# ztaylor797/APMBackend

Measured on AMD Instinct MI355X. Metric: log-lines/sec z-scored (whole node), higher is better.
Workload: dtype fp64

## Files before the change

### apmbackend_amd/csrc/bindings.cpp

```cpp
#include <pybind11/pybind11.h>
#include <pybind11/stl.h>

#include <cstring>
#include <memory>

#include "kernels/kernel_api.h"
#include "runtime/engine.h"
#include "runtime/format.h"
#include "runtime/jsutil.h"
#include "runtime/merge.h"

namespace apm {
namespace copyenc {
void encode_blob(std::string_view blob, std::string* out, int64_t* counts);
}
int apm_txcopy_lines(const char* d_text, const uint64_t* h_line_off, int64_t n, std::string& out_rows);
std::vector<double> apm_release_bench(int64_t n, int iters, uint64_t seed);
}

namespace py = pybind11;
using namespace apm;

void register_tailer(py::module_& m);
void register_synth(py::module_& m);
// ... 759 lines not shown
  m.def("js_parse_int", [](const std::string& s) { return js::parse_int(s); });
  m.def("js_convert_date", [](const std::string& s, const py::dict& tz) {
    double v;
    TzTable t = tz_from(tz);
    if (!js::convert_date(s, t, v)) return py::object(py::none());
    return py::object(py::float_(v));
  });
  m.def("js_round_fixed", [](double x, int f) { return js_round_fixed(x, f); });
  m.def("hist_bin", [](int32_t v) { return hist_bin(v); });
  m.def("hist_lower", [](int b) { return hist_lower(b); });
  m.def("hist_group_max", []() { return apm_hist_group_max(); });
  m.def("winpct_group_max", []() { return apm_winpct_group_max(); });
  m.def("winpct_group_win", []() { return apm_winpct_group_win(); });
  m.def("slo_group_max", []() { return apm_slo_group_max(); });
  m.def("slo_stage_bytes", []() { return apm_slo_stage_bytes(); });

  register_tailer(m);
  register_synth(m);
  register_procstat(m);
  register_dbsink(m);
}
```

### apmbackend_amd/csrc/kernels/devjoin.hip

```cpp
#include "kernel_api.h"

#include <rocprim/rocprim.hpp>

#include <chrono>
#include <climits>
#include <cstdlib>
#include <cstddef>
#include <cstring>
#include <vector>

#include "devjoin_api.h"
#include "devjoin_dev.h"
#include "devscan.h"
#include "prim.h"
#include "textout.h"

namespace apm {
using namespace dj;

namespace {

constexpr int TB = 256;

__device__ __forceinline__ uint32_t grid_n(uint32_t n) { return (n + TB - 1) / TB; }
// ... 2271 lines not shown
}
static int dj_scan_bucket_max(PrimScratch& sc, const int64_t* bucket, int64_t* bmax, size_t n, hipStream_t s) {
  return prim_inclusive_scan(sc, bucket, bmax, n, rocprim::maximum<int64_t>(), s);
}

size_t apm_dj_tmp_bytes(uint32_t max_ev, uint32_t max_out) {
  PrimScratch q;
  const size_t n = std::max<size_t>(max_ev, 1) + 1;
  dj_sort_keys(q, nullptr, nullptr, nullptr, nullptr, n, 0);
  dj_scan_counts(q, nullptr, nullptr, n, 0);
  dj_scan_lens(q, nullptr, nullptr, (size_t)max_out + 1, 0);
  dj_scan_bucket_max(q, nullptr, nullptr, (size_t)max_out + 1, 0);
  return q.need + 4096;
}

int apm_dj_select_host(DJArgs* a, const uint32_t* d_n_ev, uint32_t max_ev, hipStream_t s) {
  HIP_OK(hipMemsetAsync(a->n_host, 0, sizeof(SelCount), s));
  if (max_ev == 0) return 0;
  uint32_t* list = reinterpret_cast<uint32_t*>(a->sel_pos);
  uint32_t* list_n = list + max_ev;
  HIP_OK(hipMemsetAsync(list_n, 0, 8, s));
  const dim3 grid((max_ev + TB - 1) / TB);
  hipLaunchKernelGGL(k_host_flags, grid, dim3(TB), 0, s, a->ev, d_n_ev, a->bytes, a->host_flag, a->sel_val, a->aud,
                     a->n_host, max_ev, list, list_n);
  dj_check(s, "k_host_flags");
  hipLaunchKernelGGL(k_host_flags_bytes, grid, dim3(TB), 0, s, a->ev, a->bytes, a->chunk_file, a->file_fkey,
                     a->host_flag, a->sel_val, a->aud, max_ev, list, list_n);
  dj_check(s, "k_host_flags_bytes");
  uint64_t* total = a->sel_pos + (max_ev + DS_TILE - 1) / DS_TILE + 1;
  if (ds_scan_apply<uint64_t>(SelValF{a->sel_val},
                              SelScatterG{a->ev, a->host_flag, total, a->host_ev, a->host_ev_idx, a->mh_idx,
                                          a->walk_idx, a->n_host},
                              d_n_ev, max_ev, a->sel_pos, total, s) != 0)
    return -1;
  dj_check(s, "k_ds_scan (host selection)");
  return 0;
// ... 337 lines not shown
```

### apmbackend_amd/csrc/kernels/devjoin_api.h

```cpp
#pragma once
#include <vector>
#include <hip/hip_runtime.h>
#include <stdint.h>

#include "../apm_types.h"
#include "devjoin_types.h"

namespace apm {

constexpr int SOAP_SEGS = 16;
constexpr uint32_t DJ_OVF_CAP = 1u << 16;

enum : uint32_t {
  DJ_WRITE_OK = 0,
  DJ_WRITE_TXT = 1,
  DJ_WRITE_TOO_BIG = 2,
  DJ_WRITE_RING_FULL = 3,
};

__host__ __device__ inline uint64_t ring_place(uint64_t head, uint64_t bytes, uint64_t cap) {
  return ((head & (cap - 1)) + bytes > cap) ? (head + cap - 1) & ~(cap - 1) : head;
}

struct DJOverflow {
// ... 138 lines not shown
  uint32_t* unresolved;
  char* txt_tx;
  char* txt_db;
  int want_tx, want_db;
  JoinCounts* counts;
  void* tmp;
  size_t tmp_bytes;
};

}

extern "C" {
size_t apm_dj_tmp_bytes(uint32_t max_ev, uint32_t max_out);
int apm_dj_take_marks(double* t, const char** names, int cap);
void apm_dj_gather_field(const void* base, size_t stride, uint32_t n, int words, uint32_t* out, hipStream_t s);
int apm_dj_select_host(apm::DJArgs* a, const uint32_t* d_n_ev, uint32_t max_ev, hipStream_t s);
int apm_dj_join(apm::DJArgs* a, hipStream_t s);
int apm_dj_plan(apm::DJFormatArgs* f, hipStream_t s);
int apm_dj_write(apm::DJFormatArgs* f, hipStream_t s);
void apm_dj_rebuild(const apm::KeyState* old, uint32_t old_cap, apm::KeyState* fresh, uint32_t fresh_mask,
                    const apm::NeedEnt* arena, uint32_t arena_cap, double now, apm::JoinCounts* counts,
                    unsigned long long* live, uint8_t* pool, uint32_t* pool_ring, uint32_t pool_mask, hipStream_t s);
size_t apm_dj_rebuild_scratch_bytes(uint32_t cap);
std::vector<double> apm_dj_rebuild_selftest(uint32_t cap, double load, double dead, uint64_t seed, bool copy);
void apm_dj_rebuild_inplace(apm::KeyState* table, uint32_t cap, uint32_t* scratch, const apm::NeedEnt* arena,
                            uint32_t arena_cap, double now, apm::JoinCounts* counts, unsigned long long* live,
                            uint8_t* pool, uint32_t* pool_ring, uint32_t pool_mask, hipStream_t s);
size_t apm_dj_live_tmp_bytes(uint32_t cap);
void apm_dj_live_compact(const apm::KeyState* table, uint32_t cap, apm::KeyState* out, uint32_t* d_n, void* tmp,
                         size_t tmp_bytes, hipStream_t s);
void apm_dj_gather_blocks(const uint8_t* pool, const int32_t* idx, uint32_t n, uint8_t* out, hipStream_t s);
// ... 28 lines not shown
```

### apmbackend_amd/csrc/kernels/kernel_api.h

```cpp
#pragma once
#include <hip/hip_runtime.h>
#include <stdint.h>

#include "../apm_types.h"
#include "common.h"

namespace apm {

struct StatsState {
  int32_t* counts;
  int32_t* cells;
  int32_t* spill_n;
  int32_t* spill_series;
  int32_t* spill_val;
  uint8_t* active;
  int32_t cap;
  int32_t spill_cap;
  int32_t S;
  int32_t nslot = NSLOT_MIN;
  unsigned long long* spill_drop = nullptr;
  int32_t* nan_until = nullptr;
  int32_t* ord_list = nullptr;
  int32_t* ord_n = nullptr;
  uint32_t* ord_done = nullptr;
// ... 62 lines not shown
};

struct CopySeg {
  void* dst;
  const void* src;
  size_t bytes;
};
struct CopySegs {
  CopySeg seg[8];
  int32_t n = 0;
  void add(void* d, const void* s, size_t b) {
    if (b) seg[n++] = CopySeg{d, s, b};
  }
};

struct ExportArgs {
  static constexpr int kMax = 8;
  void* src[kMax];
  void* dst[kMax];
  uint64_t reset_val[kMax];
  uint8_t bytes[kMax];
  uint8_t reset[kMax];
  int32_t n;
  void add(void* s, void* d, int nb, bool rst = false, uint64_t rv = 0) {
    src[n] = s; dst[n] = d; bytes[n] = (uint8_t)nb; reset[n] = rst ? 1 : 0; reset_val[n] = rv; ++n;
  }
};

struct FormatArgs {
  const int32_t* perm;
// ... 124 lines not shown
  int32_t both_only;
  int32_t max_out;
  const double* cool_t;
  double now;
  double cool_s;
};

}

extern "C" {
size_t apm_parse_workspace_bytes(uint64_t max_bytes, uint32_t max_lines, uint32_t max_chunks);
int apm_parse_batch(const uint8_t* d_bytes, uint64_t n_bytes, const uint32_t* d_chunk_begin,
                    const uint8_t* d_chunk_kind, const uint32_t* d_chunk_file, uint32_t n_chunks,
                    void* d_ws, uint32_t max_lines, apm::Event* d_events, uint32_t* d_n_events,
                    uint32_t* d_n_lines, unsigned long long* d_watermark, uint8_t* d_file_open,
                    const apm::TzTable* tz, hipStream_t stream);
size_t apm_ck_pack_tmp_bytes(uint64_t n_entries);
int apm_ck_pack_cells(const int32_t* counts, const int32_t* cells, const int32_t* d_slots, int k, int32_t n, int32_t S,
                      int32_t cap, uint32_t* lens, uint32_t* offs, void* tmp, size_t tmp_bytes, int32_t* packed,
                      hipStream_t s);
void apm_stats_clear_slot(apm::StatsState* st, int slot, hipStream_t stream);
void apm_bucket_append(const apm::TxRec* d_tx, uint32_t lo, uint32_t hi, apm::StatsState* st,
                       int64_t min_live_bucket, hipStream_t stream);
void apm_nan_mark(const apm::TxRec* d_tx, uint32_t n, apm::StatsState* st, hipStream_t stream);
void apm_window_stats(apm::WindowArgs* a, hipStream_t stream);
size_t apm_spill_sort_tmp_bytes(int32_t spill_cap, int32_t S, int32_t nslot);
int apm_spill_sort(const apm::StatsState* st, int32_t* series_out, int32_t* val_out, void* tmp, size_t tmp_bytes,
                   hipStream_t stream);
void apm_pool_append(const apm::TxRec* d_tx, uint32_t lo, uint32_t hi, const int64_t* d_gid, int64_t* tail_end,
                     int64_t* tail_gid, int64_t base, hipStream_t stream);
size_t apm_release_tmp_bytes(int64_t cap);
// ... 56 lines not shown
```

### apmbackend_amd/csrc/kernels/parse.hip

```cpp
#include "kernel_api.h"

#include "prim.h"

#include "devscan.h"

#include <algorithm>
#include <cstdio>
#include <cstdlib>
#include <cstring>

namespace apm {

constexpr int NL_BLOCK = 256;
constexpr int NL_TILE = NL_BLOCK * 16;
constexpr int PARSE_BLOCK = 256;
constexpr int PARSE_LDS = 32 * 1024;

constexpr int NL_PER = 4;

__device__ __forceinline__ uint32_t nl_count16(const uint4 v) {
  const uint32_t w[4] = {v.x, v.y, v.z, v.w};
  uint32_t c = 0;
#pragma unroll
  for (int k = 0; k < 4; ++k) {
    const uint32_t x = w[k] ^ 0x0a0a0a0aU;
    const uint32_t t = ~(((x & 0x7F7F7F7Fu) + 0x7F7F7F7Fu) | x | 0x7F7F7F7Fu);
    c += __popc(t);
  }
  return c;
}

__global__ __launch_bounds__(NL_BLOCK) void k_nl_count(const uint8_t* __restrict__ bytes, uint64_t n,
                                                      uint32_t* __restrict__ tile_counts, uint8_t* __restrict__ pad,
                                                      uint32_t tiles) {
  if (blockIdx.x == 0 && threadIdx.x < 64) pad[threadIdx.x] = 0;
  if (blockIdx.x == 0 && threadIdx.x == 64) tile_counts[tiles] = 0;
  uint4 v[NL_PER];
  uint64_t base[NL_PER];
#pragma unroll
  for (int k = 0; k < NL_PER; ++k) {
    base[k] = ((uint64_t)blockIdx.x * NL_PER + k) * NL_TILE + threadIdx.x * 16;
    if (base[k] + 16 <= n) v[k] = *reinterpret_cast<const uint4*>(bytes + base[k]);
  }
  uint32_t pk[NL_PER / 2] = {0, 0};
#pragma unroll
  for (int k = 0; k < NL_PER; ++k) {
    uint32_t c = 0;
    if (base[k] + 16 <= n) {
      c = nl_count16(v[k]);
    } else {
      for (uint64_t i = base[k]; i < n && i < base[k] + 16; ++i) c += bytes[i] == '\n';
// ... 2 lines not shown
  }
  __shared__ uint32_t red[NL_PER / 2][NL_BLOCK / APM_WAVE];
#pragma unroll
  for (int h = 0; h < NL_PER / 2; ++h) {
    uint32_t c = pk[h];
    for (int o = 32; o > 0; o >>= 1) c += __shfl_down(c, o, APM_WAVE);
    if ((threadIdx.x & 63) == 0) red[h][threadIdx.x >> 6] = c;
  }
  __syncthreads();
  if (threadIdx.x < NL_PER) {
    const int k = threadIdx.x;
    uint32_t sum = 0;
    for (int i = 0; i < NL_BLOCK / APM_WAVE; ++i) sum += red[k >> 1][i];
    const uint32_t tile = blockIdx.x * NL_PER + k;
    if (tile < tiles) tile_counts[tile] = (sum >> (16 * (k & 1))) & 0xFFFFu;
  }
}

__global__ __launch_bounds__(NL_BLOCK) void k_nl_write(const uint8_t* __restrict__ bytes, uint64_t n,
                                                      const uint32_t* __restrict__ tile_off,
                                                      uint32_t* __restrict__ line_end, uint32_t* __restrict__ n_lines,
                                                      uint32_t tiles) {
  if (blockIdx.x == 0 && threadIdx.x == 0) *n_lines = tile_off[tiles];
  uint4 v[NL_PER];
#pragma unroll
  for (int k = 0; k < NL_PER; ++k) {
    const uint64_t base = ((uint64_t)blockIdx.x * NL_PER + k) * NL_TILE + threadIdx.x * 16;
    v[k] = base + 16 <= n ? *reinterpret_cast<const uint4*>(bytes + base) : make_uint4(0, 0, 0, 0);
  }
  typedef rocprim::block_scan<int, NL_BLOCK> Scan;
// ... 941 lines not shown
  __device__ uint32_t operator()(uint32_t i) const { return keep[i]; }
};
struct CompactG {
  const uint8_t* keep;
  const Event* ev_tmp;
  Event* out;
  __device__ void operator()(uint32_t i, uint32_t p) const {
    if (keep[i]) out[p] = ev_tmp[i];
  }
};

}

extern "C" {

constexpr size_t APM_SCAN_TMP = 32u << 20;

size_t apm_parse_workspace_bytes(uint64_t max_bytes, uint32_t max_lines, uint32_t max_chunks) {
  using namespace apm;
  const uint64_t tiles = (max_bytes + NL_TILE - 1) / NL_TILE + 2;
  size_t b = 0;
  b += tiles * 8 + 64;
  b += (size_t)max_lines * (4 + 4 + 4 + 1) + 64;
  b += (size_t)max_lines * sizeof(Event) + 64;
  b += (size_t)(max_chunks + 2) * 4 + 256;
  b += (size_t)(max_chunks + 2) * (SEC_SEGS + 1) + 256;
  b += APM_SCAN_TMP;
  return b;
}

int apm_parse_batch(const uint8_t* d_bytes, uint64_t n_bytes, const uint32_t* d_chunk_begin,
                    const uint8_t* d_chunk_kind, const uint32_t* d_chunk_file, uint32_t n_chunks,
                    void* d_ws, uint32_t max_lines, apm::Event* d_events, uint32_t* d_n_events,
                    uint32_t* d_n_lines, unsigned long long* d_watermark, uint8_t* d_file_open,
                    const apm::TzTable* tz, hipStream_t stream) {
  using namespace apm;
  const uint32_t tiles = (uint32_t)((n_bytes + NL_TILE - 1) / NL_TILE);
  if (tiles == 0 || n_chunks == 0) {
    HIP_OK(hipMemsetAsync(d_n_events, 0, 4, stream));
    HIP_OK(hipMemsetAsync(d_n_lines, 0, 4, stream));
    HIP_OK(hipMemsetAsync(const_cast<uint8_t*>(d_bytes) + n_bytes, 0, 64, stream));
    return 0;
  }
  const uint32_t cap = (uint32_t)std::min<uint64_t>(max_lines, n_bytes);
  uint8_t* w = (uint8_t*)d_ws;
  auto carve = [&](size_t bytes) { uint8_t* r = (uint8_t*)(((uintptr_t)w + 63) & ~(uintptr_t)63); w = r + bytes; return r; };
  uint32_t* tile_counts = (uint32_t*)carve((size_t)(tiles + 1) * 4);
  uint32_t* tile_off = (uint32_t*)carve((size_t)(tiles + 1) * 4);
  uint32_t* line_end = (uint32_t*)carve((size_t)max_lines * 4);
  Event* ev_tmp = (Event*)carve((size_t)max_lines * sizeof(Event));
  uint32_t* line_mask = (uint32_t*)carve((size_t)max_lines * 4);
  uint32_t* pos = (uint32_t*)carve((size_t)max_lines * 4);
  uint8_t* keep = carve((size_t)max_lines);
  uint32_t* chunk_line_lo = (uint32_t*)carve((size_t)(n_chunks + 2) * 4);
  uint8_t* seg_state = carve((size_t)(n_chunks + 2) * SEC_SEGS);
  uint8_t* chunk_init = carve((size_t)(n_chunks + 2));
  void* scan_tmp = carve(APM_SCAN_TMP);

  const uint32_t nl_blocks = (tiles + NL_PER - 1) / NL_PER;
  hipLaunchKernelGGL(k_nl_count, dim3(nl_blocks), dim3(NL_BLOCK), 0, stream, d_bytes, n_bytes, tile_counts,
                     const_cast<uint8_t*>(d_bytes) + n_bytes, tiles);
  PrimScratch sc(scan_tmp, APM_SCAN_TMP);
  if (prim_exclusive_scan(sc, tile_counts, tile_off, 0u, (size_t)tiles + 1, rocprim::plus<uint32_t>(), stream) != 0)
    return -1;
  hipLaunchKernelGGL(k_nl_write, dim3(nl_blocks), dim3(NL_BLOCK), 0, stream, d_bytes, n_bytes, tile_off, line_end,
                     d_n_lines, tiles);

  ParseArgs pa;
  pa.bytes = d_bytes;
  pa.line_end = line_end;
  pa.chunk_begin = d_chunk_begin;
  pa.chunk_kind = d_chunk_kind;
  pa.n_lines_dev = d_n_lines;
  pa.cap_lines = cap;
  pa.n_chunks = n_chunks;
  pa.ev_tmp = ev_tmp;
  pa.line_mask = line_mask;
  pa.keep = keep;
  pa.watermark = d_watermark;
// ... 25 lines not shown
            h[PP_COOP] ? (double)h[PP_HEAD] / h[PP_COOP] : 0.0, h[PP_COOP] ? (double)h[PP_TAIL] / h[PP_COOP] : 0.0);
  }
  hipLaunchKernelGGL(k_chunk_lines, dim3((n_chunks + 1 + 255) / 256), dim3(256), 0, stream, d_chunk_begin,
                     n_chunks, line_end, d_n_lines, chunk_line_lo, tile_off, tiles);
  hipLaunchKernelGGL(k_section_summary, dim3(n_chunks, SEC_SEGS), dim3(APM_WAVE), 0, stream, chunk_line_lo,
                     d_chunk_kind, d_chunk_file, n_chunks, line_mask, d_file_open, seg_state, chunk_init);
  hipLaunchKernelGGL(k_section_apply, dim3(n_chunks, SEC_SEGS), dim3(APM_WAVE), 0, stream, chunk_line_lo,
                     d_chunk_kind, d_chunk_file, n_chunks, line_mask, keep, ev_tmp, d_file_open, seg_state,
                     chunk_init);
  if (ds_scan_apply<uint32_t>(KeepF{keep}, CompactG{keep, ev_tmp, d_events}, d_n_lines, cap, pos, d_n_events,
                              stream) != 0)
    return -1;
  return 0;
}

}
```

### apmbackend_amd/csrc/runtime/devjoin.cpp

```cpp
#include "devjoin.h"

#include <algorithm>
#include <chrono>
#include <climits>
#include <cstddef>
#include <cstdlib>
#include <cstring>
#include <stdexcept>

#include "../kernels/common.h"
#include "binio.h"
#include "d2h.h"
#include "../kernels/devjoin_dev.h"
#include "../kernels/kernel_api.h"
#include "join_util.h"
#include "jsutil.h"

namespace apm {

using namespace jstr;

namespace {
double clock_ms() {
  return std::chrono::duration<double, std::milli>(std::chrono::steady_clock::now().time_since_epoch()).count();
// ... 38 lines not shown
    s.host_flag = (uint8_t*)res_.dmalloc_on(stream_, E + 64);
    s.d_host_ev = (Event*)res_.dmalloc_on(stream_, (size_t)E * sizeof(Event));
    s.d_host_idx = (uint32_t*)res_.dmalloc_on(stream_, (size_t)E * 4);
    s.d_mh_idx = (uint32_t*)res_.dmalloc_on(stream_, (size_t)E * 4);
    s.d_walk_idx = (uint32_t*)res_.dmalloc_on(stream_, (size_t)E * 4);
    s.d_aud = (AudF*)res_.dmalloc_on(stream_, (size_t)E * sizeof(AudF));
    s.d_n_host = (SelCount*)res_.dmalloc_on(stream_, 64);
    res_.pin(s.h_host_ev, (size_t)E * sizeof(Event));
    res_.pin(s.h_host_idx, (size_t)E * 4);
    res_.pin(s.h_n_host, 64);
    std::memset(s.h_n_host, 0, 64);
    s.d_chunk_next = (int32_t*)res_.dmalloc_on(stream_, ((size_t)cfg_.max_chunks + 2) * 4);
    s.d_chunk_first = (uint8_t*)res_.dmalloc_on(stream_, (size_t)cfg_.max_chunks + 2);
    res_.pin(s.h_chunk_next, ((size_t)cfg_.max_chunks + 2) * 4);
    res_.pin(s.h_chunk_first, (size_t)cfg_.max_chunks + 2);
    s.d_tx = (TxRec*)res_.dmalloc_on(stream_, (size_t)out_cap_ * sizeof(TxRec));
    s.d_tx_raw = (int32_t*)res_.dmalloc_on(stream_, (size_t)out_cap_ * 4);
    s.d_tx_gid = (int64_t*)res_.dmalloc_on(stream_, (size_t)out_cap_ * 8);
    s.free_ev = res_.new_event();
  }
  table_cap_ = 1u << cfg_.table_bits;
  init_table_cap_ = table_cap_;
  init_arena_cap_ = cfg_.arena_cap;
  d_table_ = (KeyState*)res_.dmalloc_on(stream_, (size_t)table_cap_ * sizeof(KeyState));
  d_reg_ = (RegSlot*)res_.dmalloc_on(stream_, ((size_t)1 << cfg_.reg_bits) * sizeof(RegSlot));
  miss_cap_ = E;
  d_miss_ = (RegMiss*)res_.dmalloc_on(stream_, (size_t)miss_cap_ * sizeof(RegMiss));
  res_.pin(h_miss_, (size_t)miss_cap_ * sizeof(RegMiss));
  d_arena_ = (NeedEnt*)res_.dmalloc_on(stream_, (size_t)cfg_.arena_cap * sizeof(NeedEnt));
  d_exp_lo_ = (uint64_t*)res_.dmalloc_on(stream_, 8 * 4096);
// ... 97 lines not shown
  const size_t n = files_->size();
  if (n <= h_file_fkey_.size()) return;
  if (n > soap_cap_) throw std::runtime_error("device join: too many files");
  const size_t lo = h_file_fkey_.size();
  if (lo == 0) HIP_OK(hipStreamSynchronize(stream_));
  for (size_t i = lo; i < n; ++i) {
    const FileInfo& f = (*files_)[i];
    const std::string& srv = (*servers_)[f.server];
    h_file_skey_.push_back(dj::server_key_of(srv.data(), srv.size()));
    h_file_fkey_.push_back(dj::file_key_of(f.path.data(), f.path.size()));
  }
  HIP_OK(hipMemcpy(d_file_skey_ + lo, h_file_skey_.data() + lo, (n - lo) * 8, hipMemcpyHostToDevice));
  HIP_OK(hipMemcpy(d_file_fkey_ + lo, h_file_fkey_.data() + lo, (n - lo) * 8, hipMemcpyHostToDevice));
}

void DeviceJoin::select_host(int k, const uint32_t* d_n_ev, uint32_t max_ev, hipStream_t ps) {
  Slot& s = sl_[k];
  sync_file_keys();
  DJArgs a{};
  a.ev = s.d_events;
  a.bytes = s.d_bytes;
  a.host_flag = s.host_flag;
  a.chunk_file = s.d_chunk_file;
  a.file_fkey = d_file_fkey_;
  a.aud = s.d_aud;
  a.sel_val = d_sel_val_;
  a.sel_pos = d_sel_pos_;
  a.host_ev = s.d_host_ev;
  a.host_ev_idx = s.d_host_idx;
  a.mh_idx = s.d_mh_idx;
  a.walk_idx = s.d_walk_idx;
  a.n_host = s.d_n_host;
  a.tmp = d_sel_tmp_;
  a.tmp_bytes = sel_tmp_bytes_;
  if (apm_dj_select_host(&a, d_n_ev, std::min<uint32_t>(max_ev, cfg_.max_events), ps) != 0)
    throw std::runtime_error("device join: scan scratch too small");
  HIP_OK(hipMemcpyAsync(s.h_n_host, s.d_n_host, sizeof(SelCount), hipMemcpyDeviceToHost, ps));
  s.spec = std::min<uint32_t>(cfg_.max_events, last_host_ + last_host_ / 4 + 256);
  HIP_OK(hipMemcpyAsync(s.h_host_ev, s.d_host_ev, (size_t)s.spec * sizeof(Event), hipMemcpyDeviceToHost, ps));
  HIP_OK(hipMemcpyAsync(s.h_host_idx, s.d_host_idx, (size_t)s.spec * 4, hipMemcpyDeviceToHost, ps));
}

void DeviceJoin::set_chunks(int k, const std::vector<int32_t>& chunk_file, const uint32_t* d_chunk_file,
                            const uint8_t* d_chunk_kind, hipStream_t ps) {
  Slot& s = sl_[k];
  const uint32_t n = (uint32_t)chunk_file.size();
  std::unordered_map<int32_t, int32_t> last;
  for (uint32_t c = 0; c < n; ++c) {
    s.h_chunk_next[c] = -1;
    auto it = last.find(chunk_file[c]);
    if (it == last.end()) {
      s.h_chunk_first[c] = 1;
    } else {
      s.h_chunk_first[c] = 0;
      s.h_chunk_next[it->second] = (int32_t)c;
    }
    last[chunk_file[c]] = (int32_t)c;
  }
  if (n) {
    HIP_OK(hipMemcpyAsync(s.d_chunk_next, s.h_chunk_next, (size_t)n * 4, hipMemcpyHostToDevice, ps));
    HIP_OK(hipMemcpyAsync(s.d_chunk_first, s.h_chunk_first, n, hipMemcpyHostToDevice, ps));
  }
  s.d_chunk_file = d_chunk_file;
  s.d_chunk_kind = d_chunk_kind;
  s.n_chunks = n;
  s.chunk_file = chunk_file;
}

void DeviceJoin::finish_select(int k, hipStream_t ps) {
  Slot& s = sl_[k];
  const uint32_t n = s.h_n_host->host;
  if (n > s.spec) {
    HIP_OK(hipMemcpyAsync(s.h_host_ev + s.spec, s.d_host_ev + s.spec, (size_t)(n - s.spec) * sizeof(Event),
                          hipMemcpyDeviceToHost, ps));
    HIP_OK(hipMemcpyAsync(s.h_host_idx + s.spec, s.d_host_idx + s.spec, (size_t)(n - s.spec) * 4,
                          hipMemcpyDeviceToHost, ps));
    HIP_OK(hipStreamSynchronize(ps));
// ... 572 lines not shown
  spans.clear();
  double sp = phase_t[1];
  auto span = [&](const char* name) { const double t = clock_ms(); spans.push_back({name, {sp, t}}); sp = t; };
  res_.reserve(h_hops_, hops_.size(), hops_.size() * 2 + 65536, true);
  res_.reserve(h_hbuf_, hbuf_.size(), hbuf_.size() * 2 + (4 << 20), true);
  span("u.hostgrow");
  if (hops_.size() > d_hops_cap_) {
    d_hops_cap_ = hops_.size() * 2 + 65536;
    d_hops_ = (HostOp*)res_.dmalloc_raw(d_hops_cap_ * sizeof(HostOp));
  }
  if (hbuf_.size() > d_hbuf_cap_) {
    d_hbuf_cap_ = hbuf_.size() * 2 + (4 << 20);
    d_hbuf_ = (uint8_t*)res_.dmalloc_raw(d_hbuf_cap_);
  }
  span("u.devgrow");
  if (!hops_.empty()) {
    std::memcpy(h_hops_, hops_.data(), hops_.size() * sizeof(HostOp));
    span("u.hops.memcpy");
    apm_copy(d_hops_, h_hops_.d, hops_.size() * sizeof(HostOp), st);
    span("u.hops.h2d");
  }
  if (!hbuf_.empty()) {
    std::memcpy(h_hbuf_, hbuf_.data(), hbuf_.size());
    span("u.hbuf.memcpy");
    apm_copy(d_hbuf_, h_hbuf_.d, hbuf_.size(), st);
    span("u.hbuf.h2d");
  }
  sync_file_keys();
  if (files_->size() > files_uploaded_) {
    if (files_->size() > soap_cap_) throw std::runtime_error("device join: too many files");
    std::vector<int32_t> fs(files_->size() - files_uploaded_);
    for (size_t i = files_uploaded_; i < files_->size(); ++i) fs[i - files_uploaded_] = (*files_)[i].server;
    HIP_OK(hipMemcpyAsync(d_file_server_ + files_uploaded_, fs.data(), fs.size() * 4, hipMemcpyHostToDevice, st));
    HIP_OK(hipStreamSynchronize(st));
    files_uploaded_ = files_->size();
  }
  ensure_capacity(n_ev, n_bytes + hbuf_.size(), now);
  span("u.capacity");
  const uint64_t arena_low = regions_.empty() ? arena_head_ : regions_.front().lo;
  const uint32_t arena_limit = (uint32_t)((uint64_t)cfg_.arena_cap - (arena_head_ - arena_low));
  uint32_t n_reg = 0, n_exp = 0;
  while (!regions_.empty() && regions_.front().exp < now && n_reg < 4096) {
    h_exp_[n_reg] = regions_.front().lo;
    h_exp_[4096 + n_reg] = regions_.front().hi;
    n_exp += (uint32_t)(regions_.front().hi - regions_.front().lo);
    regions_.pop_front();
    ++n_reg;
  }
  if (n_reg) {
    apm_copy(d_exp_lo_, h_exp_.d, (size_t)n_reg * 8, st);
    apm_copy(d_exp_hi_, (const uint64_t*)h_exp_.d + 4096, (size_t)n_reg * 8, st);
  }
  span("u.files+exp");
  DJArgs& a = a_;
  a = DJArgs{};
  a.ev = s.d_events; a.n_ev = n_ev; a.bytes = s.d_bytes;
  a.chunk_file = s.d_chunk_file; a.chunk_kind = s.d_chunk_kind; a.n_chunks = s.n_chunks;
  a.chunk_next = s.d_chunk_next; a.chunk_first = s.d_chunk_first; a.file_server = d_file_server_;
  a.file_skey = d_file_skey_; a.file_fkey = d_file_fkey_;
  a.hops = d_hops_; a.n_hops = (uint32_t)hops_.size(); a.hbuf = d_hbuf_;
  a.now = now; a.batch_no = batch_no;
  a.rec_ttl = cfg_.record_ttl_ms; a.acct_ttl = cfg_.acct_ttl_ms; a.need_ttl = cfg_.need_ttl_ms;
  a.host_flag = s.host_flag;
  a.ops = d_ops_; a.soap_code = d_soap_code_; a.soap_num = d_soap_num_; a.soap_hash = d_soap_hash_;
  a.chunk_ev_lo = d_chunk_ev_lo_; a.seg_f = d_seg_f_; a.seg_in = d_seg_in_; a.chain_hash = d_chain_hash_;
  a.soap_state = d_soap_;
  a.op_slot = d_op_slot_; a.op_slot_sorted = d_op_slot_sorted_; a.op_idx = d_op_idx_; a.op_idx_sorted = d_op_idx_sorted_;
// ... 668 lines not shown
```

### apmbackend_amd/csrc/runtime/devjoin.h

```cpp
#pragma once
#include <hip/hip_runtime.h>

#include <atomic>
#include <cstdint>
#include <deque>
#include <functional>
#include <mutex>
#include <string>
#include <unordered_map>
#include <vector>

#include "../apm_types.h"
#include "../kernels/devjoin_api.h"
#include "hipres.h"
#include "join.h"

namespace apm {

struct DevJoinConfig {
  uint32_t max_events = 1u << 20;
  uint64_t max_batch_bytes = 64ull << 20;
  uint32_t max_chunks = 4096;
  int table_bits = 21;
  int reg_bits = 20;
  uint32_t max_raw = 1u << 20;
  uint32_t arena_cap = 1u << 20;
  uint32_t pool_blocks = 0;
  uint64_t ring_bytes = 4ull << 30;
// ... 19 lines not shown
 public:
  DeviceJoin(const DevJoinConfig& cfg, Dictionary* dict, const std::vector<FileInfo>* files,
             const std::vector<std::string>* servers);
  ~DeviceJoin();

  uint8_t* d_bytes(int k) { return sl_[k].d_bytes; }
  uint8_t* d_stage() {
    if (!d_stage_bytes_) {
      d_stage_bytes_ = (uint8_t*)res_.dmalloc_on(stream_, cfg_.max_batch_bytes + 256);
      HIP_OK(hipStreamSynchronize(stream_));
    }
    return d_stage_bytes_;
  }
  void swap_stage(int k) { std::swap(sl_[k].d_bytes, d_stage_bytes_); }
  Event* d_events(int k) { return sl_[k].d_events; }
  void select_host(int k, const uint32_t* d_n_ev, uint32_t max_ev, hipStream_t ps);
  void set_chunks(int k, const std::vector<int32_t>& chunk_file, const uint32_t* d_chunk_file,
                  const uint8_t* d_chunk_kind, hipStream_t ps);
  void finish_select(int k, hipStream_t ps);
  using ParallelFor = std::function<void(int, const std::function<void(int)>&)>;
  void run(int k, const uint8_t* host_bytes, uint32_t n_ev, uint64_t n_bytes, double now, uint64_t batch_no, bool want_tx,
           bool want_db, DevJoinBatch& out, const ParallelFor& parallel = nullptr,
           const std::function<void()>* meanwhile = nullptr);
  void prepass_ahead(int k, const uint8_t* host_bytes, const ParallelFor& parallel);
  void release_slot(int k, hipStream_t stats_stream);

  int32_t raw_server(int32_t raw) const { return raw_info_[raw].server; }
  int32_t raw_service(int32_t raw) const { return raw_info_[raw].norm_id; }
  int32_t n_raw() const { return n_raw_.load(std::memory_order_acquire); }
  int32_t* d_raw_series() { return d_raw_series_; }

  char* ring() { return d_ring_; }
  uint64_t ring_cap() const { return cfg_.ring_bytes; }
// ... 25 lines not shown
    uint8_t* host_flag = nullptr;
    Event* d_host_ev = nullptr;
    uint32_t* d_host_idx = nullptr;
    uint32_t* d_mh_idx = nullptr;
    uint32_t* d_walk_idx = nullptr;
    AudF* d_aud = nullptr;
    SelCount* d_n_host = nullptr;
    Event* h_host_ev = nullptr;
    uint32_t* h_host_idx = nullptr;
    SelCount* h_n_host = nullptr;
    uint32_t spec = 0;
    int32_t* d_chunk_next = nullptr;
    uint8_t* d_chunk_first = nullptr;
    int32_t* h_chunk_next = nullptr;
    uint8_t* h_chunk_first = nullptr;
    const uint32_t* d_chunk_file = nullptr;
    const uint8_t* d_chunk_kind = nullptr;
    uint32_t n_chunks = 0;
    std::vector<int32_t> chunk_file;
    TxRec* d_tx = nullptr;
    int32_t* d_tx_raw = nullptr;
    int64_t* d_tx_gid = nullptr;
    hipEvent_t free_ev = nullptr;
    bool used = false;
  } sl_[2];

  struct RawInfo { int32_t server; int32_t norm_id; uint64_t svc; };

  struct PrepassTask {
    int32_t file = -1;
// ... 174 lines not shown
```

### apmbackend_amd/csrc/runtime/engine.cpp

```cpp
#include <cstdlib>
#include "engine.h"

#include <pthread.h>
#include <sched.h>

#include <cctype>
#include <fstream>

#include <rocprofiler-sdk-roctx/roctx.h>

#include <unistd.h>

#include <cerrno>
#include <cstring>

#include <algorithm>
#include <exception>
#include <chrono>
#include <cmath>
#include <cstring>
#include <queue>
#include <stdexcept>

#include "../kernels/devjoin_api.h"
// ... 259 lines not shown
    res_.pin(h_unseen_flag_, (size_t)cfg_.max_series);
  } else {
    d_bytes_ = (uint8_t*)res_.dmalloc(cfg_.max_batch_bytes + 256);
  }
  for (int k = 0; k < 2; ++k) {
    ParseSlot& ps = pslot_[k];
    res_.pin(ps.h_bytes, cfg_.max_batch_bytes + 256);
    res_.pin(ps.h_chunk_begin, (cfg_.max_chunks + 2) * 4);
    res_.pin(ps.h_chunk_kind, cfg_.max_chunks + 2);
    res_.pin(ps.h_chunk_file, (cfg_.max_chunks + 2) * 4);
    d_chunk_begin_[k] = (uint32_t*)res_.dmalloc((cfg_.max_chunks + 2) * 4);
    d_chunk_kind_[k] = (uint8_t*)res_.dmalloc(cfg_.max_chunks + 2);
    d_chunk_file_[k] = (uint32_t*)res_.dmalloc((cfg_.max_chunks + 2) * 4);
    res_.pin(ps.h_counts, 16);
    res_.pin(ps.h_watermark, 8);
    if (dev()) continue;
    res_.pin(ps.h_events, (size_t)cfg_.max_lines * sizeof(Event));
  }
  d_parse_ws_ = res_.dmalloc(apm_parse_workspace_bytes(cfg_.max_batch_bytes, cfg_.max_lines, cfg_.max_chunks));
  if (!dev()) d_events_ = (Event*)res_.dmalloc((size_t)cfg_.max_lines * sizeof(Event));
  d_counts_ = (uint32_t*)res_.dmalloc(16);
  d_watermark_ = (unsigned long long*)res_.dmalloc(8);
  d_file_open_ = (uint8_t*)res_.dmalloc(1 << 16);
  init_spill_cap_ = cfg_.spill_cap;
  alloc_ring(std::max(cfg_.nslot, ring_slots_for(cfg_.window, cfg_.buffer)));
  for (auto& m : spill_mark_) m.ev = res_.new_event();
  metrics_.spill_capacity = cfg_.spill_cap;
  d_spill_drop_ = (unsigned long long*)res_.dmalloc(64);
  d_active_ = (uint8_t*)res_.dmalloc(S);
  d_win_ = (WinStat*)res_.dmalloc((size_t)S * sizeof(WinStat));
// ... 481 lines not shown
  ++metrics_.batches;

  const int k = (int)(&ps - pslot_);
  bool staged = false;
  if (dev() && canonical && in_stage_src_ == host_bytes && in_stage_n_ == n_bytes && in_stage_ev_) {
    HIP_OK(hipStreamWaitEvent(parse_stream_, in_stage_ev_, 0));
    dj_->swap_stage(k);
    staged = true;
    ++metrics_.staged_batches;
  }
  in_stage_src_ = nullptr;
  in_stage_n_ = 0;
  uint8_t* dbytes = dev() ? dj_->d_bytes(k) : d_bytes_;
  Event* devents = dev() ? dj_->d_events(k) : d_events_;
  if (!staged) HIP_OK(hipMemcpyAsync(dbytes, ps.hb, off, hipMemcpyHostToDevice, parse_stream_));
  h2d(d_chunk_begin_[k], ps.h_chunk_begin, (n_chunks + 1) * 4, parse_stream_);
  h2d(d_chunk_kind_[k], ps.h_chunk_kind, n_chunks + 1, parse_stream_);
  h2d(d_chunk_file_[k], ps.h_chunk_file, (n_chunks + 1) * 4, parse_stream_);
  if (apm_parse_batch(dbytes, off, d_chunk_begin_[k], d_chunk_kind_[k], d_chunk_file_[k], n_chunks, d_parse_ws_,
                      cfg_.max_lines, devents, d_counts_, d_counts_ + 1, d_watermark_, d_file_open_, &cfg_.tz,
                      parse_stream_) != 0)
    throw std::runtime_error("parse workspace too small");
  if (dev()) {
    dj_->set_chunks(k, ps.chunk_file, d_chunk_file_[k], d_chunk_kind_[k], parse_stream_);
    dj_->select_host(k, d_counts_, cfg_.max_lines, parse_stream_);
  }
  d2h(ps.h_counts, d_counts_, 8, parse_stream_);
  d2h(ps.h_watermark, d_watermark_, 8, parse_stream_);
  ps.spec_copied = 0;
  if (speculative && !dev() && spec_events_) {
    ps.spec_copied = std::min<uint32_t>(spec_events_, cfg_.max_lines);
    HIP_OK(hipMemcpyAsync(ps.h_events, d_events_, (size_t)ps.spec_copied * sizeof(Event), hipMemcpyDeviceToHost,
                          parse_stream_));
  }
  ps.pending = true;
  metrics_.t_parse_ms += now_ms() - t0;
}

void Engine::stage_batch(const uint8_t* host_bytes, uint64_t n_bytes) {
  if (!dev() || !host_bytes || n_bytes == 0 || n_bytes > cfg_.max_batch_bytes) return;
  const double t0 = now_ms();
  if (!in_stage_stream_) {
    HIP_OK(hipStreamCreateWithFlags(&in_stage_stream_, hipStreamNonBlocking));
// ... 2778 lines not shown
```

### apmbackend_amd/csrc/runtime/engine.h

```cpp
#pragma once
#include <hip/hip_runtime.h>

#include "binio.h"

#include <array>
#include <atomic>
#include <condition_variable>
#include <cstdint>
#include <deque>
#include <functional>
#include <map>
#include <memory>
#include <mutex>
#include <string>
#include <thread>
#include <unordered_map>
#include <vector>

#include "../apm_types.h"
#include "../kernels/kernel_api.h"
#include "collective.h"
#include "devjoin.h"
#include "hipres.h"
#include "join.h"
// ... 617 lines not shown
  int32_t* d_unseen_idx_ = nullptr;
  uint8_t* d_unseen_flag_ = nullptr;
  uint8_t* h_unseen_flag_ = nullptr;
  unsigned long long* d_unmapped_ = nullptr;
  bool dev() const { return dj_ != nullptr; }

  uint8_t* d_bytes_ = nullptr;
  struct ParseSlot {
    uint8_t* h_bytes = nullptr;
    uint32_t* h_chunk_begin = nullptr;
    uint8_t* h_chunk_kind = nullptr;
    uint32_t* h_chunk_file = nullptr;
    Event* h_events = nullptr;
    uint32_t* h_counts = nullptr;
    unsigned long long* h_watermark = nullptr;
    const uint8_t* hb = nullptr;
    const uint8_t* src = nullptr;
    uint64_t src_n = 0, n_bytes = 0;
    std::vector<int32_t> chunk_file;
    uint32_t n_events = 0, n_lines = 0;
    uint32_t spec_copied = 0;
    bool pending = false;
  } pslot_[2];
  uint32_t spec_events_ = 0;
  int cur_slot_ = 0, last_slot_ = 0;
  bool prefetched_ = false;
  const uint8_t* in_stage_src_ = nullptr;
  uint64_t in_stage_n_ = 0;
  hipStream_t in_stage_stream_ = nullptr;
  hipEvent_t in_stage_ev_ = nullptr;
// ... 379 lines not shown
```

Measured before the change: 301.3 million.

## Batch parse-path small copies, fold memsets into nl_count, use single-block tile scan

Several small host-device copies in the parse launch path (chunk metadata, select counts, watermark) are gathered into batched copy-segment launches that use device aliases of the pinned host buffers. The memsets for the host-selection counters are folded into the first block of the newline-count kernel. The rocprim device scan over tile counts is replaced by a single 1024-thread block scan kernel, which also drops the 32MB scan scratch. The aim is fewer launches and less API overhead per batch. The cost is that the single-block scan runs serially for large tile counts, and the copy ordering has changed: set_chunks now uploads before parse rather than after it.

```diff
diff --git a/apmbackend_amd/csrc/bindings.cpp b/apmbackend_amd/csrc/bindings.cpp
--- a/apmbackend_amd/csrc/bindings.cpp
+++ b/apmbackend_amd/csrc/bindings.cpp
@@ -797,6 +797,20 @@
   m.def("winpct_group_win", []() { return apm_winpct_group_win(); });
   m.def("slo_group_max", []() { return apm_slo_group_max(); });
   m.def("slo_stage_bytes", []() { return apm_slo_stage_bytes(); });
+  m.def("tile_scan_block", []() { return apm_tile_scan_block(); });
+  m.def("gpu_tile_scan", [](py::bytes counts) {
+    const std::string in = counts;
+    if (in.size() % 4) throw std::invalid_argument("gpu_tile_scan: whole uint32 words");
+    const size_t n = in.size() / 4;
+    if (n > 0xFFFF0000u) throw std::invalid_argument("gpu_tile_scan: too many entries");
+    std::string out(n * 4, '\0');
+    if (n == 0) return py::bytes(out);
+    DevMem din(n * 4), dout(n * 4);
+    HIP_OK(hipMemcpy(din.p, in.data(), n * 4, hipMemcpyHostToDevice));
+    apm_tile_scan(din.as<uint32_t>(), dout.as<uint32_t>(), (uint32_t)n, 0);
+    HIP_OK(hipMemcpy(out.data(), dout.p, n * 4, hipMemcpyDeviceToHost));
+    return py::bytes(out);
+  }, py::arg("counts"));
 
   register_tailer(m);
   register_synth(m);
diff --git a/apmbackend_amd/csrc/kernels/devjoin.hip b/apmbackend_amd/csrc/kernels/devjoin.hip
--- a/apmbackend_amd/csrc/kernels/devjoin.hip
+++ b/apmbackend_amd/csrc/kernels/devjoin.hip
@@ -2309,12 +2309,16 @@
   return q.need + 4096;
 }
 
-int apm_dj_select_host(DJArgs* a, const uint32_t* d_n_ev, uint32_t max_ev, hipStream_t s) {
-  HIP_OK(hipMemsetAsync(a->n_host, 0, sizeof(SelCount), s));
+uint32_t* apm_dj_select_list_counts(uint64_t* sel_pos, uint32_t max_ev) {
+  return reinterpret_cast<uint32_t*>(sel_pos) + max_ev;
+}
+
+int apm_dj_select_host(DJArgs* a, const uint32_t* d_n_ev, uint32_t max_ev, hipStream_t s, bool prezeroed) {
+  if (!prezeroed) HIP_OK(hipMemsetAsync(a->n_host, 0, sizeof(SelCount), s));
   if (max_ev == 0) return 0;
   uint32_t* list = reinterpret_cast<uint32_t*>(a->sel_pos);
-  uint32_t* list_n = list + max_ev;
-  HIP_OK(hipMemsetAsync(list_n, 0, 8, s));
+  uint32_t* list_n = apm_dj_select_list_counts(a->sel_pos, max_ev);
+  if (!prezeroed) HIP_OK(hipMemsetAsync(list_n, 0, 8, s));
   const dim3 grid((max_ev + TB - 1) / TB);
   hipLaunchKernelGGL(k_host_flags, grid, dim3(TB), 0, s, a->ev, d_n_ev, a->bytes, a->host_flag, a->sel_val, a->aud,
                      a->n_host, max_ev, list, list_n);
diff --git a/apmbackend_amd/csrc/kernels/devjoin_api.h b/apmbackend_amd/csrc/kernels/devjoin_api.h
--- a/apmbackend_amd/csrc/kernels/devjoin_api.h
+++ b/apmbackend_amd/csrc/kernels/devjoin_api.h
@@ -176,7 +176,9 @@
 size_t apm_dj_tmp_bytes(uint32_t max_ev, uint32_t max_out);
 int apm_dj_take_marks(double* t, const char** names, int cap);
 void apm_dj_gather_field(const void* base, size_t stride, uint32_t n, int words, uint32_t* out, hipStream_t s);
-int apm_dj_select_host(apm::DJArgs* a, const uint32_t* d_n_ev, uint32_t max_ev, hipStream_t s);
+int apm_dj_select_host(apm::DJArgs* a, const uint32_t* d_n_ev, uint32_t max_ev, hipStream_t s,
+                       bool prezeroed = false);
+uint32_t* apm_dj_select_list_counts(uint64_t* sel_pos, uint32_t max_ev);
 int apm_dj_join(apm::DJArgs* a, hipStream_t s);
 int apm_dj_plan(apm::DJFormatArgs* f, hipStream_t s);
 int apm_dj_write(apm::DJFormatArgs* f, hipStream_t s);
diff --git a/apmbackend_amd/csrc/kernels/kernel_api.h b/apmbackend_amd/csrc/kernels/kernel_api.h
--- a/apmbackend_amd/csrc/kernels/kernel_api.h
+++ b/apmbackend_amd/csrc/kernels/kernel_api.h
@@ -100,6 +100,16 @@
   }
 };
 
+struct ParseZero {
+  static constexpr int kMax = 2;
+  uint32_t* p[kMax];
+  uint32_t words[kMax];
+  int32_t n = 0;
+  void add(void* d, uint32_t w) {
+    if (w) { p[n] = (uint32_t*)d; words[n] = w; ++n; }
+  }
+};
+
 struct ExportArgs {
   static constexpr int kMax = 8;
   void* src[kMax];
@@ -254,7 +264,9 @@
                     const uint8_t* d_chunk_kind, const uint32_t* d_chunk_file, uint32_t n_chunks,
                     void* d_ws, uint32_t max_lines, apm::Event* d_events, uint32_t* d_n_events,
                     uint32_t* d_n_lines, unsigned long long* d_watermark, uint8_t* d_file_open,
-                    const apm::TzTable* tz, hipStream_t stream);
+                    const apm::TzTable* tz, hipStream_t stream, const apm::ParseZero* zero = nullptr);
+void apm_tile_scan(const uint32_t* d_in, uint32_t* d_out, uint32_t n, hipStream_t stream);
+int apm_tile_scan_block();
 size_t apm_ck_pack_tmp_bytes(uint64_t n_entries);
 int apm_ck_pack_cells(const int32_t* counts, const int32_t* cells, const int32_t* d_slots, int k, int32_t n, int32_t S,
                       int32_t cap, uint32_t* lens, uint32_t* offs, void* tmp, size_t tmp_bytes, int32_t* packed,
diff --git a/apmbackend_amd/csrc/kernels/parse.hip b/apmbackend_amd/csrc/kernels/parse.hip
--- a/apmbackend_amd/csrc/kernels/parse.hip
+++ b/apmbackend_amd/csrc/kernels/parse.hip
@@ -1,6 +1,4 @@
 #include "kernel_api.h"
-
-#include "prim.h"
 
 #include "devscan.h"
 
@@ -32,9 +30,14 @@
 
 __global__ __launch_bounds__(NL_BLOCK) void k_nl_count(const uint8_t* __restrict__ bytes, uint64_t n,
                                                       uint32_t* __restrict__ tile_counts, uint8_t* __restrict__ pad,
-                                                      uint32_t tiles) {
+                                                      uint32_t tiles, ParseZero z) {
   if (blockIdx.x == 0 && threadIdx.x < 64) pad[threadIdx.x] = 0;
   if (blockIdx.x == 0 && threadIdx.x == 64) tile_counts[tiles] = 0;
+  if (blockIdx.x == 0) {
+#pragma unroll
+    for (int j = 0; j < ParseZero::kMax; ++j)
+      if (threadIdx.x < z.words[j]) z.p[j][threadIdx.x] = 0;
+  }
   uint4 v[NL_PER];
   uint64_t base[NL_PER];
 #pragma unroll
@@ -67,6 +70,27 @@
     for (int i = 0; i < NL_BLOCK / APM_WAVE; ++i) sum += red[k >> 1][i];
     const uint32_t tile = blockIdx.x * NL_PER + k;
     if (tile < tiles) tile_counts[tile] = (sum >> (16 * (k & 1))) & 0xFFFFu;
+  }
+}
+
+constexpr int TS_BLOCK = 1024;
+
+__global__ __launch_bounds__(TS_BLOCK) void k_tile_scan(const uint32_t* __restrict__ in, uint32_t* __restrict__ out,
+                                                        uint32_t n) {
+  typedef rocprim::block_scan<uint32_t, TS_BLOCK> Scan;
+  __shared__ typename Scan::storage_type st;
+  uint32_t carry = 0;
+  uint32_t v = threadIdx.x < n ? in[threadIdx.x] : 0u;
+  for (uint32_t base = 0; base < n; base += TS_BLOCK) {
+    const uint32_t i = base + threadIdx.x;
+    const uint32_t nx = i + TS_BLOCK;
+    const uint32_t vn = nx < n ? in[nx] : 0u;
+    uint32_t excl, sum;
+    Scan().exclusive_scan(v, excl, 0u, sum, st);
+    if (i < n) out[i] = carry + excl;
+    carry += sum;
+    v = vn;
+    __syncthreads();
   }
 }
 
@@ -1038,8 +1062,6 @@
 
 extern "C" {
 
-constexpr size_t APM_SCAN_TMP = 32u << 20;
-
 size_t apm_parse_workspace_bytes(uint64_t max_bytes, uint32_t max_lines, uint32_t max_chunks) {
   using namespace apm;
   const uint64_t tiles = (max_bytes + NL_TILE - 1) / NL_TILE + 2;
@@ -1049,7 +1071,6 @@
   b += (size_t)max_lines * sizeof(Event) + 64;
   b += (size_t)(max_chunks + 2) * 4 + 256;
   b += (size_t)(max_chunks + 2) * (SEC_SEGS + 1) + 256;
-  b += APM_SCAN_TMP;
   return b;
 }
 
@@ -1057,10 +1078,16 @@
                     const uint8_t* d_chunk_kind, const uint32_t* d_chunk_file, uint32_t n_chunks,
                     void* d_ws, uint32_t max_lines, apm::Event* d_events, uint32_t* d_n_events,
                     uint32_t* d_n_lines, unsigned long long* d_watermark, uint8_t* d_file_open,
-                    const apm::TzTable* tz, hipStream_t stream) {
+                    const apm::TzTable* tz, hipStream_t stream, const apm::ParseZero* zero) {
   using namespace apm;
   const uint32_t tiles = (uint32_t)((n_bytes + NL_TILE - 1) / NL_TILE);
+  ParseZero z{};
+  if (zero) z = *zero;
+  for (int j = 0; j < ParseZero::kMax; ++j)
+    if (z.words[j] > (uint32_t)NL_BLOCK) return -1;
   if (tiles == 0 || n_chunks == 0) {
+    for (int j = 0; j < ParseZero::kMax; ++j)
+      if (z.words[j]) HIP_OK(hipMemsetAsync(z.p[j], 0, (size_t)z.words[j] * 4, stream));
     HIP_OK(hipMemsetAsync(d_n_events, 0, 4, stream));
     HIP_OK(hipMemsetAsync(d_n_lines, 0, 4, stream));
     HIP_OK(hipMemsetAsync(const_cast<uint8_t*>(d_bytes) + n_bytes, 0, 64, stream));
@@ -1079,14 +1106,12 @@
   uint32_t* chunk_line_lo = (uint32_t*)carve((size_t)(n_chunks + 2) * 4);
   uint8_t* seg_state = carve((size_t)(n_chunks + 2) * SEC_SEGS);
   uint8_t* chunk_init = carve((size_t)(n_chunks + 2));
-  void* scan_tmp = carve(APM_SCAN_TMP);
 
   const uint32_t nl_blocks = (tiles + NL_PER - 1) / NL_PER;
   hipLaunchKernelGGL(k_nl_count, dim3(nl_blocks), dim3(NL_BLOCK), 0, stream, d_bytes, n_bytes, tile_counts,
-                     const_cast<uint8_t*>(d_bytes) + n_bytes, tiles);
-  PrimScratch sc(scan_tmp, APM_SCAN_TMP);
-  if (prim_exclusive_scan(sc, tile_counts, tile_off, 0u, (size_t)tiles + 1, rocprim::plus<uint32_t>(), stream) != 0)
-    return -1;
+                     const_cast<uint8_t*>(d_bytes) + n_bytes, tiles, z);
+  hipLaunchKernelGGL(k_tile_scan, dim3(1), dim3(TS_BLOCK), 0, stream, (const uint32_t*)tile_counts, tile_off,
+                     tiles + 1);
   hipLaunchKernelGGL(k_nl_write, dim3(nl_blocks), dim3(NL_BLOCK), 0, stream, d_bytes, n_bytes, tile_off, line_end,
                      d_n_lines, tiles);
 
@@ -1142,4 +1167,10 @@
   return 0;
 }
 
-}
+int apm_tile_scan_block() { return apm::TS_BLOCK; }
+
+void apm_tile_scan(const uint32_t* d_in, uint32_t* d_out, uint32_t n, hipStream_t stream) {
+  hipLaunchKernelGGL(apm::k_tile_scan, dim3(1), dim3(apm::TS_BLOCK), 0, stream, d_in, d_out, n);
+}
+
+}
diff --git a/apmbackend_amd/csrc/runtime/devjoin.cpp b/apmbackend_amd/csrc/runtime/devjoin.cpp
--- a/apmbackend_amd/csrc/runtime/devjoin.cpp
+++ b/apmbackend_amd/csrc/runtime/devjoin.cpp
@@ -76,6 +76,9 @@
     s.d_chunk_first = (uint8_t*)res_.dmalloc_on(stream_, (size_t)cfg_.max_chunks + 2);
     res_.pin(s.h_chunk_next, ((size_t)cfg_.max_chunks + 2) * 4);
     res_.pin(s.h_chunk_first, (size_t)cfg_.max_chunks + 2);
+    s.a_n_host = HipRes::device_alias(s.h_n_host);
+    s.a_chunk_next = HipRes::device_alias(s.h_chunk_next);
+    s.a_chunk_first = HipRes::device_alias(s.h_chunk_first);
     s.d_tx = (TxRec*)res_.dmalloc_on(stream_, (size_t)out_cap_ * sizeof(TxRec));
     s.d_tx_raw = (int32_t*)res_.dmalloc_on(stream_, (size_t)out_cap_ * 4);
     s.d_tx_gid = (int64_t*)res_.dmalloc_on(stream_, (size_t)out_cap_ * 8);
@@ -203,7 +206,14 @@
   HIP_OK(hipMemcpy(d_file_fkey_ + lo, h_file_fkey_.data() + lo, (n - lo) * 8, hipMemcpyHostToDevice));
 }
 
-void DeviceJoin::select_host(int k, const uint32_t* d_n_ev, uint32_t max_ev, hipStream_t ps) {
+void DeviceJoin::select_zero(int k, uint32_t max_ev, ParseZero& z) {
+  static_assert(sizeof(SelCount) % 4 == 0, "SelCount words");
+  z.add(sl_[k].d_n_host, (uint32_t)(sizeof(SelCount) / 4));
+  const uint32_t m = std::min<uint32_t>(max_ev, cfg_.max_events);
+  if (m) z.add(apm_dj_select_list_counts(d_sel_pos_, m), 2);
+}
+
+void DeviceJoin::select_host(int k, const uint32_t* d_n_ev, uint32_t max_ev, hipStream_t ps, CopySegs& back) {
   Slot& s = sl_[k];
   sync_file_keys();
   DJArgs a{};
@@ -222,16 +232,16 @@
   a.n_host = s.d_n_host;
   a.tmp = d_sel_tmp_;
   a.tmp_bytes = sel_tmp_bytes_;
-  if (apm_dj_select_host(&a, d_n_ev, std::min<uint32_t>(max_ev, cfg_.max_events), ps) != 0)
+  if (apm_dj_select_host(&a, d_n_ev, std::min<uint32_t>(max_ev, cfg_.max_events), ps, true) != 0)
     throw std::runtime_error("device join: scan scratch too small");
-  HIP_OK(hipMemcpyAsync(s.h_n_host, s.d_n_host, sizeof(SelCount), hipMemcpyDeviceToHost, ps));
+  back.add(s.a_n_host, s.d_n_host, sizeof(SelCount));
   s.spec = std::min<uint32_t>(cfg_.max_events, last_host_ + last_host_ / 4 + 256);
   HIP_OK(hipMemcpyAsync(s.h_host_ev, s.d_host_ev, (size_t)s.spec * sizeof(Event), hipMemcpyDeviceToHost, ps));
   HIP_OK(hipMemcpyAsync(s.h_host_idx, s.d_host_idx, (size_t)s.spec * 4, hipMemcpyDeviceToHost, ps));
 }
 
 void DeviceJoin::set_chunks(int k, const std::vector<int32_t>& chunk_file, const uint32_t* d_chunk_file,
-                            const uint8_t* d_chunk_kind, hipStream_t ps) {
+                            const uint8_t* d_chunk_kind, CopySegs& up) {
   Slot& s = sl_[k];
   const uint32_t n = (uint32_t)chunk_file.size();
   std::unordered_map<int32_t, int32_t> last;
@@ -246,10 +256,8 @@
     }
     last[chunk_file[c]] = (int32_t)c;
   }
-  if (n) {
-    HIP_OK(hipMemcpyAsync(s.d_chunk_next, s.h_chunk_next, (size_t)n * 4, hipMemcpyHostToDevice, ps));
-    HIP_OK(hipMemcpyAsync(s.d_chunk_first, s.h_chunk_first, n, hipMemcpyHostToDevice, ps));
-  }
+  up.add(s.d_chunk_next, s.a_chunk_next, (size_t)n * 4);
+  up.add(s.d_chunk_first, s.a_chunk_first, n);
   s.d_chunk_file = d_chunk_file;
   s.d_chunk_kind = d_chunk_kind;
   s.n_chunks = n;
@@ -852,18 +860,19 @@
     d_hbuf_ = (uint8_t*)res_.dmalloc_raw(d_hbuf_cap_);
   }
   span("u.devgrow");
+  CopySegs up;
   if (!hops_.empty()) {
     std::memcpy(h_hops_, hops_.data(), hops_.size() * sizeof(HostOp));
     span("u.hops.memcpy");
-    apm_copy(d_hops_, h_hops_.d, hops_.size() * sizeof(HostOp), st);
-    span("u.hops.h2d");
+    up.add(d_hops_, h_hops_.d, hops_.size() * sizeof(HostOp));
   }
   if (!hbuf_.empty()) {
     std::memcpy(h_hbuf_, hbuf_.data(), hbuf_.size());
     span("u.hbuf.memcpy");
-    apm_copy(d_hbuf_, h_hbuf_.d, hbuf_.size(), st);
-    span("u.hbuf.h2d");
-  }
+    up.add(d_hbuf_, h_hbuf_.d, hbuf_.size());
+  }
+  apm_copy_segs(&up, st);
+  span("u.h2d");
   sync_file_keys();
   if (files_->size() > files_uploaded_) {
     if (files_->size() > soap_cap_) throw std::runtime_error("device join: too many files");
@@ -885,10 +894,10 @@
     regions_.pop_front();
     ++n_reg;
   }
-  if (n_reg) {
-    apm_copy(d_exp_lo_, h_exp_.d, (size_t)n_reg * 8, st);
-    apm_copy(d_exp_hi_, (const uint64_t*)h_exp_.d + 4096, (size_t)n_reg * 8, st);
-  }
+  CopySegs up_exp;
+  up_exp.add(d_exp_lo_, h_exp_.d, (size_t)n_reg * 8);
+  up_exp.add(d_exp_hi_, (const uint64_t*)h_exp_.d + 4096, (size_t)n_reg * 8);
+  apm_copy_segs(&up_exp, st);
   span("u.files+exp");
   DJArgs& a = a_;
   a = DJArgs{};
diff --git a/apmbackend_amd/csrc/runtime/devjoin.h b/apmbackend_amd/csrc/runtime/devjoin.h
--- a/apmbackend_amd/csrc/runtime/devjoin.h
+++ b/apmbackend_amd/csrc/runtime/devjoin.h
@@ -12,6 +12,7 @@
 
 #include "../apm_types.h"
 #include "../kernels/devjoin_api.h"
+#include "../kernels/kernel_api.h"
 #include "hipres.h"
 #include "join.h"
 
@@ -61,9 +62,10 @@
   }
   void swap_stage(int k) { std::swap(sl_[k].d_bytes, d_stage_bytes_); }
   Event* d_events(int k) { return sl_[k].d_events; }
-  void select_host(int k, const uint32_t* d_n_ev, uint32_t max_ev, hipStream_t ps);
+  void select_zero(int k, uint32_t max_ev, apm::ParseZero& z);
+  void select_host(int k, const uint32_t* d_n_ev, uint32_t max_ev, hipStream_t ps, apm::CopySegs& back);
   void set_chunks(int k, const std::vector<int32_t>& chunk_file, const uint32_t* d_chunk_file,
-                  const uint8_t* d_chunk_kind, hipStream_t ps);
+                  const uint8_t* d_chunk_kind, apm::CopySegs& up);
   void finish_select(int k, hipStream_t ps);
   using ParallelFor = std::function<void(int, const std::function<void(int)>&)>;
   void run(int k, const uint8_t* host_bytes, uint32_t n_ev, uint64_t n_bytes, double now, uint64_t batch_no, bool want_tx,
@@ -119,6 +121,7 @@
     uint8_t* d_chunk_first = nullptr;
     int32_t* h_chunk_next = nullptr;
     uint8_t* h_chunk_first = nullptr;
+    void *a_n_host = nullptr, *a_chunk_next = nullptr, *a_chunk_first = nullptr;
     const uint32_t* d_chunk_file = nullptr;
     const uint8_t* d_chunk_kind = nullptr;
     uint32_t n_chunks = 0;
diff --git a/apmbackend_amd/csrc/runtime/engine.cpp b/apmbackend_amd/csrc/runtime/engine.cpp
--- a/apmbackend_amd/csrc/runtime/engine.cpp
+++ b/apmbackend_amd/csrc/runtime/engine.cpp
@@ -297,6 +297,11 @@
     d_chunk_file_[k] = (uint32_t*)res_.dmalloc((cfg_.max_chunks + 2) * 4);
     res_.pin(ps.h_counts, 16);
     res_.pin(ps.h_watermark, 8);
+    ps.a_chunk_begin = HipRes::device_alias(ps.h_chunk_begin);
+    ps.a_chunk_kind = HipRes::device_alias(ps.h_chunk_kind);
+    ps.a_chunk_file = HipRes::device_alias(ps.h_chunk_file);
+    ps.a_counts = HipRes::device_alias(ps.h_counts);
+    ps.a_watermark = HipRes::device_alias(ps.h_watermark);
     if (dev()) continue;
     res_.pin(ps.h_events, (size_t)cfg_.max_lines * sizeof(Event));
   }
@@ -808,19 +813,23 @@
   uint8_t* dbytes = dev() ? dj_->d_bytes(k) : d_bytes_;
   Event* devents = dev() ? dj_->d_events(k) : d_events_;
   if (!staged) HIP_OK(hipMemcpyAsync(dbytes, ps.hb, off, hipMemcpyHostToDevice, parse_stream_));
-  h2d(d_chunk_begin_[k], ps.h_chunk_begin, (n_chunks + 1) * 4, parse_stream_);
-  h2d(d_chunk_kind_[k], ps.h_chunk_kind, n_chunks + 1, parse_stream_);
-  h2d(d_chunk_file_[k], ps.h_chunk_file, (n_chunks + 1) * 4, parse_stream_);
+  CopySegs up;
+  up.add(d_chunk_begin_[k], ps.a_chunk_begin, (size_t)(n_chunks + 1) * 4);
+  up.add(d_chunk_kind_[k], ps.a_chunk_kind, (size_t)n_chunks + 1);
+  up.add(d_chunk_file_[k], ps.a_chunk_file, (size_t)(n_chunks + 1) * 4);
+  if (dev()) dj_->set_chunks(k, ps.chunk_file, d_chunk_file_[k], d_chunk_kind_[k], up);
+  apm_copy_segs(&up, parse_stream_);
+  ParseZero zero{};
+  if (dev()) dj_->select_zero(k, cfg_.max_lines, zero);
   if (apm_parse_batch(dbytes, off, d_chunk_begin_[k], d_chunk_kind_[k], d_chunk_file_[k], n_chunks, d_parse_ws_,
                       cfg_.max_lines, devents, d_counts_, d_counts_ + 1, d_watermark_, d_file_open_, &cfg_.tz,
-                      parse_stream_) != 0)
+                      parse_stream_, &zero) != 0)
     throw std::runtime_error("parse workspace too small");
-  if (dev()) {
-    dj_->set_chunks(k, ps.chunk_file, d_chunk_file_[k], d_chunk_kind_[k], parse_stream_);
-    dj_->select_host(k, d_counts_, cfg_.max_lines, parse_stream_);
-  }
-  d2h(ps.h_counts, d_counts_, 8, parse_stream_);
-  d2h(ps.h_watermark, d_watermark_, 8, parse_stream_);
+  CopySegs back;
+  if (dev()) dj_->select_host(k, d_counts_, cfg_.max_lines, parse_stream_, back);
+  back.add(ps.a_counts, d_counts_, 8);
+  back.add(ps.a_watermark, d_watermark_, 8);
+  apm_copy_segs(&back, parse_stream_);
   ps.spec_copied = 0;
   if (speculative && !dev() && spec_events_) {
     ps.spec_copied = std::min<uint32_t>(spec_events_, cfg_.max_lines);
diff --git a/apmbackend_amd/csrc/runtime/engine.h b/apmbackend_amd/csrc/runtime/engine.h
--- a/apmbackend_amd/csrc/runtime/engine.h
+++ b/apmbackend_amd/csrc/runtime/engine.h
@@ -655,6 +655,8 @@
     Event* h_events = nullptr;
     uint32_t* h_counts = nullptr;
     unsigned long long* h_watermark = nullptr;
+    void *a_chunk_begin = nullptr, *a_chunk_kind = nullptr, *a_chunk_file = nullptr;
+    void *a_counts = nullptr, *a_watermark = nullptr;
     const uint8_t* hb = nullptr;
     const uint8_t* src = nullptr;
     uint64_t src_n = 0, n_bytes = 0;
```

New measurement: 292.1 million. -3.0%, worse.
